# linhthi/BLISS-GNN

Hardware: AMD Instinct MI355X
Metric: steps/sec (train step: sample_blocks + gather + SAGE fwd/bwd + Adam + exp3), reddit-like (higher is better)
Workload: dtype bf16

## Files before the change

bliss_gnn_amd/csrc/sage.hip:

```cpp
#include "common.cuh"
#include "bliss_gnn.h"
#include <cstdlib>

namespace {

typedef __bf16 bf16x8_t __attribute__((ext_vector_type(8)));
typedef float f32x16_t __attribute__((ext_vector_type(16)));

#define TG_TPB 512
#define TG_M 32
#define TG_WAVES (TG_TPB / 64)
#define TG_NB (256 / 32 / TG_WAVES)

struct TileGemm {
  const bf16_t* a1; long long a1_stride; const int* ids;
  const bf16_t* w1; long long w1_stride; int k1;
  const bf16_t* a2; long long a2_stride; const bf16_t* w2; long long w2_stride; int k2;
  const bf16_t* bias;
  int m_bound; const int* m_dev; int n;
  bf16_t* out; long long out_stride;
  bf16_t* a_copy; long long copy_stride;
  bf16_t* in_norm; bf16_t* out_norm;
  int relu; unsigned drop_thresh; float drop_scale; unsigned seed; unsigned long long* ctr;
};

__device__ __forceinline__ int k_pad16(int k) { return (k + 15) & ~15; }
__device__ __host__ __forceinline__ int lds_stride(int k) {
  return ((k + 15) & ~15) + 8;
}

__device__ __forceinline__ uint32_t tg_drop_hash(uint32_t seed, uint32_t ctr, uint32_t idx) {
  uint32_t x = idx * 0x9e3779b1u + seed;
  x ^= ctr * 0x85ebca77u + 0x165667b1u;
  x ^= x >> 16; x *= 0x7feb352du; x ^= x >> 15; x *= 0x846ca68bu; x ^= x >> 16;
  x += ctr; x ^= x >> 15; x *= 0x2c1b3c6du; x ^= x >> 12;
  return x;
}

__device__ __forceinline__ float row_sumsq(const bf16_t* sh, int dim, int vec4, int lane) {
  float s = 0.f;
  if (vec4) {
    for (int c = lane * 4; c < dim; c += 256) {
      const float a = bf2f(sh[c]), b = bf2f(sh[c + 1]), cc = bf2f(sh[c + 2]), d = bf2f(sh[c + 3]);
      s += a * a; s += b * b; s += cc * cc; s += d * d;
    }
  } else {
    for (int c = lane; c < dim; c += 64) { const float a = bf2f(sh[c]); s += a * a; }
  }
  for (int d = 32; d >= 1; d >>= 1) s += __shfl_xor(s, d);
  return s;
}

__device__ __forceinline__ void rows_norm(const bf16_t* tile, int stride, int dim, int row0, int M, int m_bound, bf16_t* __restrict__ out,
                                          int wave, int lane) {
  constexpr int RPW = TG_M / TG_WAVES;
  float s[RPW];
#pragma unroll
  for (int q = 0; q < RPW; ++q) s[q] = 0.f;
  if (dim % 4 == 0) {
    for (int c = lane * 4; c < dim; c += 256)
#pragma unroll
      for (int q = 0; q < RPW; ++q) {
        const bf16_t* sh = tile + (size_t)(q * TG_WAVES + wave) * stride + c;
        const float a = bf2f(sh[0]), b = bf2f(sh[1]), cc = bf2f(sh[2]), d = bf2f(sh[3]);
        s[q] += a * a; s[q] += b * b; s[q] += cc * cc; s[q] += d * d;
      }
  } else {
    for (int c = lane; c < dim; c += 64)
#pragma unroll
      for (int q = 0; q < RPW; ++q) { const float a = bf2f(tile[(size_t)(q * TG_WAVES + wave) * stride + c]); s[q] += a * a; }
  }
  for (int d = 32; d >= 1; d >>= 1)
#pragma unroll
    for (int q = 0; q < RPW; ++q) s[q] += __shfl_xor(s[q], d);
#pragma unroll
  for (int q = 0; q < RPW; ++q) {
    const int r = row0 + q * TG_WAVES + wave;
    if (lane == 0 && r < m_bound) out[r] = r < M ? f2bf(sqrtf(s[q])) : (bf16_t)0;
  }
}

__device__ __forceinline__ void stage_rows(const bf16_t* __restrict__ a, long long a_stride, const int* row_id, int k,
                                           int row0, int m_bound, bf16_t* tile, int stride, bf16_t* __restrict__ copy, long long copy_stride,
                                           int wave, int lane) {
  const int kp = k_pad16(k);
  const bool even = (k % 2 == 0) && (a_stride % 2 == 0) && (((uintptr_t)a) % 4 == 0);
  const bool copy32 = copy && (copy_stride % 2 == 0) && (((uintptr_t)copy) % 4 == 0);
  if (even) {
    const int dw = k / 2;
    constexpr int MAXC = (1024 / 2 + 63) / 64;
    constexpr int RPW = TG_M / TG_WAVES, HALF = RPW;
#pragma unroll
    for (int hb = 0; hb < 1; ++hb) {
      uint32_t v[HALF][MAXC];
#pragma unroll
      for (int q = 0; q < HALF; ++q) {
        const int id = row_id[(hb * HALF + q) * TG_WAVES + wave];
        const uint32_t* src = reinterpret_cast<const uint32_t*>(a + (long long)(id < 0 ? 0 : id) * a_stride);
#pragma unroll
        for (int j = 0; j < MAXC; ++j) {
          const int c = lane + 64 * j;
          const uint32_t x = src[c < dw ? c : dw - 1];
          v[q][j] = (id >= 0 && c < dw) ? x : 0u;
        }
      }
#pragma unroll
      for (int q = 0; q < HALF; ++q) {
        const int lr = (hb * HALF + q) * TG_WAVES + wave, r = row0 + lr;
        uint32_t* sh = reinterpret_cast<uint32_t*>(tile + (size_t)lr * stride);
#pragma unroll
        for (int j = 0; j < MAXC; ++j) {
          const int c = lane + 64 * j;
          if (c < kp / 2) sh[c] = v[q][j];
          if (copy && r < m_bound && c < dw) {
            if (copy32) reinterpret_cast<uint32_t*>(copy + (long long)r * copy_stride)[c] = v[q][j];
            else { bf16_t* cp = copy + (long long)r * copy_stride + 2 * c; cp[0] = (bf16_t)(v[q][j] & 0xffffu); cp[1] = (bf16_t)(v[q][j] >> 16); }
          }
        }
      }
    }
  } else {
    for (int rd = 0; rd < TG_M / TG_WAVES; ++rd) {
      const int lr = rd * TG_WAVES + wave, r = row0 + lr, id = row_id[lr];
      const bf16_t* src = a + (long long)(id < 0 ? 0 : id) * a_stride;
      bf16_t* sh = tile + (size_t)lr * stride;
      for (int c = lane; c < kp; c += 64) {
        const bf16_t x = (id >= 0 && c < k) ? src[c] : (bf16_t)0;
        sh[c] = x;
        if (copy && r < m_bound && c < k) copy[(long long)r * copy_stride + c] = x;
      }
    }
  }
}

#define TG_SLAB 64
#define TG_WSTRIDE (TG_SLAB + 8)
#define TG_WROWS 256
typedef uint32_t u32x4_a4 __attribute__((ext_vector_type(4), aligned(4)));

struct WRegs { uint4 v[TG_WROWS * TG_SLAB / 8 / TG_TPB]; };

__device__ __forceinline__ void w_slab_load_full(WRegs& g, const bf16_t* __restrict__ w, long long w_stride, int N, int slab, int tid) {
  const int part = tid & 7, k = slab * TG_SLAB + 8 * part;
#pragma unroll
  for (int i = 0; i < (int)(sizeof(g.v) / sizeof(g.v[0])); ++i) {
    int n = i * (TG_TPB / 8) + (tid >> 3);
    n = n < N ? n : N - 1;
    const u32x4_a4 q = *reinterpret_cast<const u32x4_a4*>(w + (long long)n * w_stride + k);
    g.v[i] = make_uint4(q[0], q[1], q[2], q[3]);
  }
}
__device__ __forceinline__ void w_slab_load_tail(WRegs& g, const bf16_t* __restrict__ w, long long w_stride, int N, int K, int slab, int tid) {
  const int part = tid & 7, k = slab * TG_SLAB + 8 * part;
  for (int i = 0; i < (int)(sizeof(g.v) / sizeof(g.v[0])); ++i) {
    int n = i * (TG_TPB / 8) + (tid >> 3);
    n = n < N ? n : N - 1;
    const bf16_t* p = w + (long long)n * w_stride + k;
    union { uint4 u; bf16_t e[8]; } t;
    t.u = make_uint4(0, 0, 0, 0);
    for (int j = 0; j < 8; ++j) if (k + j < K) t.e[j] = p[j];
    g.v[i] = t.u;
  }
}
__device__ __forceinline__ int w_full_slabs(const bf16_t* w, long long w_stride, int K) {
  return ((w_stride % 2 == 0) && (((uintptr_t)w) % 4 == 0)) ? K / TG_SLAB : 0;
}
__device__ __forceinline__ void w_slab_store(const WRegs& g, bf16_t* wl, int tid) {
  const int part = tid & 7;
#pragma unroll
  for (int i = 0; i < (int)(sizeof(g.v) / sizeof(g.v[0])); ++i) {
    const int n = i * (TG_TPB / 8) + (tid >> 3);
    *reinterpret_cast<uint4*>(wl + (size_t)n * TG_WSTRIDE + 8 * part) = g.v[i];
  }
}

__device__ __forceinline__ void mma_product(WRegs& ga, WRegs& gb, const bf16_t* tile, int stride, int k, const bf16_t* __restrict__ w,
                                            long long w_stride, int n0, int N, bf16_t* wl, int tid, int lane, f32x16_t acc[TG_NB]) {
  const int kp = k_pad16(k), r = lane & 31, h = lane >> 5;
  const int nslab = (kp + TG_SLAB - 1) / TG_SLAB;
  auto multiply = [&](int sl) {
    if (n0 < N) {
#pragma unroll
      for (int st = 0; st < TG_SLAB / 16; ++st) {
        const int ks = sl * TG_SLAB + 16 * st;
        if (ks < kp) {
          const bf16x8_t a = *reinterpret_cast<const bf16x8_t*>(tile + (size_t)r * stride + ks + 8 * h);
#pragma unroll
          for (int nb = 0; nb < TG_NB; ++nb) {
            const bf16x8_t b = *reinterpret_cast<const bf16x8_t*>(wl + (size_t)(n0 + 32 * nb + r) * TG_WSTRIDE + 16 * st + 8 * h);
            acc[nb] = __builtin_amdgcn_mfma_f32_32x32x16_bf16(a, b, acc[nb], 0, 0, 0);
          }
        }
      }
    }
  };
  const int nfull = w_full_slabs(w, w_stride, k);
  for (int sl = 0; sl < nfull; sl += 2) {
    __syncthreads();
    w_slab_store(ga, wl, tid);
    if (sl + 2 < nfull) w_slab_load_full(ga, w, w_stride, N, sl + 2, tid);
    __syncthreads();
    multiply(sl);
    if (sl + 1 < nfull) {
      __syncthreads();
      w_slab_store(gb, wl, tid);
      if (sl + 3 < nfull) w_slab_load_full(gb, w, w_stride, N, sl + 3, tid);
      __syncthreads();
      multiply(sl + 1);
    }
  }
  for (int sl = nfull; sl < nslab; ++sl) {
    WRegs t;
    w_slab_load_tail(t, w, w_stride, N, k, sl, tid);
    __syncthreads();
    w_slab_store(t, wl, tid);
    __syncthreads();
    multiply(sl);
  }
}

__device__ __forceinline__ void tile_gemm_body(const TileGemm& p, bf16_t* lds, int* row_id, int dbg) {
  const int tid = threadIdx.x, wave = tid >> 6, lane = tid & 63;
  int M = p.m_bound;
  if (p.m_dev) { const int t = *p.m_dev; M = t < M ? t : M; }
  const int row0 = blockIdx.x * TG_M;
  const uint32_t ctr = p.drop_thresh ? (uint32_t)__hip_atomic_load(p.ctr, __ATOMIC_RELAXED, __HIP_MEMORY_SCOPE_AGENT) : 0u;
  const int N = p.n;
  if (row0 >= p.m_bound) return;
  if (row0 >= M) {
    for (int lr = wave; lr < TG_M; lr += TG_WAVES) {
      const int r = row0 + lr;
      if (r >= p.m_bound) break;
      for (int c = lane; c < N; c += 64) p.out[(long long)r * p.out_stride + c] = 0;
      if (p.a_copy) for (int c = lane; c < p.k1; c += 64) p.a_copy[(long long)r * p.copy_stride + c] = 0;
      if (lane == 0) { if (p.in_norm) p.in_norm[r] = 0; if (p.out_norm) p.out_norm[r] = 0; }
    }
    return;
  }
  const int s1 = lds_stride(p.k1), s2 = p.k2 ? lds_stride(p.k2) : 0;
  bf16_t* t1 = lds;
  bf16_t* t2 = lds + (size_t)TG_M * s1;
  const int n0 = wave * 32 * TG_NB;
  bf16_t* wl = lds + (size_t)TG_M * (s1 + s2);
  float bias_v[TG_NB];
#pragma unroll
  for (int nb = 0; nb < TG_NB; ++nb) bias_v[nb] = 0.f;
#pragma unroll
  for (int nb = 0; nb < TG_NB; ++nb) { const int col = n0 + 32 * nb + (lane & 31); if (p.bias && col < N) bias_v[nb] = bf2f(p.bias[col]); }
  WRegs ga, gb;
  {
    const int nf = w_full_slabs(p.w1, p.w1_stride, p.k1);
    if (nf > 0) w_slab_load_full(ga, p.w1, p.w1_stride, N, 0, tid);
    if (nf > 1) w_slab_load_full(gb, p.w1, p.w1_stride, N, 1, tid);
  }
  if (tid < TG_M) {
    const int r = row0 + tid;
    row_id[tid] = r < M ? (p.ids ? p.ids[r] : r) : -1;
    row_id[TG_M + tid] = r < M ? r : -1;
  }
  __syncthreads();
  if (!(dbg & 1)) stage_rows(p.a1, p.a1_stride, row_id, p.k1, row0, p.m_bound, t1, s1, p.a_copy, p.copy_stride, wave, lane);
  if (p.k2) stage_rows(p.a2, p.a2_stride, row_id + TG_M, p.k2, row0, p.m_bound, t2, s2, nullptr, 0, wave, lane);
  __syncthreads();
  if (p.in_norm && !(dbg & 4)) rows_norm(t1, s1, p.k1, row0, M, p.m_bound, p.in_norm, wave, lane);
  f32x16_t acc[TG_NB];
#pragma unroll
  for (int m = 0; m < TG_NB; ++m)
#pragma unroll
    for (int i = 0; i < 16; ++i) acc[m][i] = 0.f;
  if (!(dbg & 2)) mma_product(ga, gb, t1, s1, p.k1, p.w1, p.w1_stride, n0, N, wl, tid, lane, acc);
  if (p.k2) {
    const int nf = w_full_slabs(p.w2, p.w2_stride, p.k2);
    if (nf > 0) w_slab_load_full(ga, p.w2, p.w2_stride, N, 0, tid);
    if (nf > 1) w_slab_load_full(gb, p.w2, p.w2_stride, N, 1, tid);
    mma_product(ga, gb, t2, s2, p.k2, p.w2, p.w2_stride, n0, N, wl, tid, lane, acc);
  }
  __syncthreads();
  const int so = ((N + 63) & ~63) + 8;
  bf16_t* ot = lds;
  if (n0 < N) {
#pragma unroll
    for (int m = 0; m < TG_NB; ++m) {
      const int col = n0 + 32 * m + (lane & 31);
      const float bv = bias_v[m];
#pragma unroll
      for (int i = 0; i < 16; ++i) {
        const int lr = (i & 3) + 8 * (i >> 2) + 4 * (lane >> 5);
        float t = rbf(acc[m][i] + bv);
        if (p.relu) t = t > 0.f ? t : 0.f;
        if (p.drop_thresh) {
          const bool keep = tg_drop_hash(p.seed, ctr, (uint32_t)((row0 + lr) * N + col)) >= p.drop_thresh;
          t = keep ? rbf(t * p.drop_scale) : 0.f;
        }
        ot[(size_t)lr * so + col] = (row0 + lr < M && col < N) ? f2bf(t) : (bf16_t)0;
      }
    }
  }
  __syncthreads();
  const bool pair_ok = (N % 2 == 0) && (p.out_stride % 2 == 0) && (((uintptr_t)p.out) % 4 == 0);
  for (int lr = wave; lr < TG_M; lr += TG_WAVES) {
    const int r = row0 + lr;
    if (r >= p.m_bound) break;
    const bf16_t* sh = ot + (size_t)lr * so;
    bf16_t* o = p.out + (long long)r * p.out_stride;
    if (pair_ok) for (int c = lane * 2; c < N; c += 128) *reinterpret_cast<uint32_t*>(o + c) = *reinterpret_cast<const uint32_t*>(sh + c);
    else for (int c = lane; c < N; c += 64) o[c] = sh[c];
  }
  if (p.out_norm) rows_norm(ot, so, N, row0, M, p.m_bound, p.out_norm, wave, lane);
}

__global__ void __launch_bounds__(TG_TPB) k_tile_gemm(TileGemm p0, TileGemm p1, int n_sets, int dbg) {
  extern __shared__ __attribute__((aligned(16))) bf16_t tg_lds[];
  __shared__ int row_id[2 * TG_M];
  if (dbg & 8) return;
  tile_gemm_body(blockIdx.y == 0 ? p0 : p1, tg_lds, row_id, dbg);
  unsigned long long* ctr = p0.drop_thresh ? p0.ctr : (n_sets > 1 && p1.drop_thresh ? p1.ctr : nullptr);
  if (ctr) {
    __syncthreads();
    if (threadIdx.x == 0) {
      const unsigned long long total = (unsigned long long)gridDim.x * gridDim.y;
      if (atomicAdd(ctr + 1, 1ull) == total - 1) {
        __hip_atomic_store(ctr + 1, 0ull, __ATOMIC_RELAXED, __HIP_MEMORY_SCOPE_AGENT);
        atomicAdd(ctr, 1ull);
      }
    }
  }
}

bool convert(const bliss_tile_gemm_t* a, TileGemm* p, size_t* lds_bytes, int* tiles) {
  if (!a->a1 || !a->w1 || !a->out || a->k1 <= 0 || a->k1 > 1024 || a->n <= 0 || a->n > 256 || a->m_bound <= 0) return false;
  if (a->k2 < 0 || a->k2 > 1024 || (a->k2 > 0 && (!a->a2 || !a->w2))) return false;
  if (a->drop_p < 0.f || a->drop_p >= 1.f || (a->drop_p > 0.f && !a->drop_ctr)) return false;
  p->a1 = (const bf16_t*)a->a1; p->a1_stride = a->a1_stride; p->ids = a->ids;
  p->w1 = (const bf16_t*)a->w1; p->w1_stride = a->w1_stride; p->k1 = a->k1;
  p->a2 = (const bf16_t*)a->a2; p->a2_stride = a->a2_stride; p->w2 = (const bf16_t*)a->w2; p->w2_stride = a->w2_stride; p->k2 = a->k2;
  p->bias = (const bf16_t*)a->bias; p->m_bound = a->m_bound; p->m_dev = a->m_dev; p->n = a->n;
  p->out = (bf16_t*)a->out; p->out_stride = a->out_stride; p->a_copy = (bf16_t*)a->a_copy; p->copy_stride = a->copy_stride;
  p->in_norm = (bf16_t*)a->in_norm; p->out_norm = (bf16_t*)a->out_norm; p->relu = a->relu;
  p->drop_thresh = a->drop_p > 0.f ? (unsigned)((double)a->drop_p * 4294967296.0) : 0u;
  p->drop_scale = a->drop_p > 0.f ? 1.0f / (1.0f - a->drop_p) : 1.0f;
  p->seed = a->drop_seed; p->ctr = (unsigned long long*)a->drop_ctr;
  const size_t stage = ((size_t)TG_M * (lds_stride(a->k1) + (a->k2 ? lds_stride(a->k2) : 0)) + (size_t)TG_WROWS * TG_WSTRIDE) * sizeof(bf16_t);
  const size_t outt = (size_t)TG_M * (((a->n + 63) & ~63) + 8) * sizeof(bf16_t);
  *lds_bytes = stage > outt ? stage : outt;
  *tiles = (a->m_bound + TG_M - 1) / TG_M;
  return true;
}

}

extern "C" int bliss_tile_gemm(const bliss_tile_gemm_t* first, const bliss_tile_gemm_t* second, void* stream) {
  if (!first) return BLISS_EINVAL;
  TileGemm p0, p1;
  size_t l0 = 0, l1 = 0;
  int t0 = 0, t1 = 0;
  if (!convert(first, &p0, &l0, &t0)) return BLISS_EINVAL;
  p1 = p0;
  if (second && !convert(second, &p1, &l1, &t1)) return BLISS_EINVAL;
  const size_t lds = l0 > l1 ? l0 : l1;
  if (lds > 160 * 1024) return BLISS_EINVAL;
  static size_t lds_set = 0;
  if (lds > lds_set) {
    if (hipFuncSetAttribute((const void*)k_tile_gemm, hipFuncAttributeMaxDynamicSharedMemorySize, (int)lds) != hipSuccess) return BLISS_EINVAL;
    lds_set = lds;
  }
  const dim3 grid(t0 > t1 ? t0 : t1, second ? 2 : 1);
  static const int dbg = []() { const char* e = getenv("BLISS_TG_DEBUG"); return e ? atoi(e) : 0; }();
  k_tile_gemm<<<grid, TG_TPB, lds, (hipStream_t)stream>>>(p0, p1, second ? 2 : 1, dbg);
  return (int)hipGetLastError();
}
```

bliss_gnn_amd/csrc/sage_bwd.hip:

```cpp
#include "common.cuh"
#include "bliss_gnn.h"
#include <cstdlib>

namespace {

typedef __bf16 bf16x8_t __attribute__((ext_vector_type(8)));
typedef short s16x4_t __attribute__((ext_vector_type(4)));
typedef short s16x8_t __attribute__((ext_vector_type(8)));
typedef float f32x16_t __attribute__((ext_vector_type(16)));
typedef uint32_t u32x4_a4 __attribute__((ext_vector_type(4), aligned(4)));

__device__ __forceinline__ s16x4_t lds_tr4(const bf16_t* p) {
  return __builtin_amdgcn_ds_read_tr16_b64_v4i16((__attribute__((address_space(3))) s16x4_t*)(p));
}
__device__ __forceinline__ bf16x8_t tr_frag(const bf16_t* img, int stride, int k0, int c0, int lane) {
  const int g = lane >> 4, i = lane & 15, q = i >> 2, p = i & 3;
  const bf16_t* a = img + (size_t)(k0 + 8 * (g >> 1) + q) * stride + c0 + 16 * (g & 1) + 4 * p;
  const s16x4_t lo = lds_tr4(a), hi = lds_tr4(a + 4 * (size_t)stride);
  s16x8_t v;
  v[0] = lo[0]; v[1] = lo[1]; v[2] = lo[2]; v[3] = lo[3]; v[4] = hi[0]; v[5] = hi[1]; v[6] = hi[2]; v[7] = hi[3];
  return __builtin_bit_cast(bf16x8_t, v);
}

__device__ __forceinline__ uint4 ld16(const bf16_t* p) {
  const u32x4_a4 q = *reinterpret_cast<const u32x4_a4*>(p);
  return make_uint4(q[0], q[1], q[2], q[3]);
}
__device__ __forceinline__ uint4 ld8_masked(const bf16_t* p, int valid, bool aligned) {
  if (valid >= 8 && aligned) return ld16(p);
  union { uint4 u; bf16_t e[8]; } t;
  t.u = make_uint4(0, 0, 0, 0);
#pragma unroll
  for (int j = 0; j < 8; ++j) if (j < valid) t.e[j] = p[j];
  return t.u;
}

#define DG_TPB 512
#define DG_M 32
#define DG_SLAB 64
#define DG_WSTRIDE (256 + 32)

struct DGrad {
  const bf16_t* a1; long long a1_stride; const bf16_t* w1; long long w1_stride; int k1;
  const bf16_t* a2; long long a2_stride; const bf16_t* w2; long long w2_stride; int k2; int m2_bound; const int* m2_dev;
  int m_bound; const int* m_dev; int n;
  bf16_t* out; long long out_stride;
};

__device__ __host__ __forceinline__ int dg_astride(int k) { return ((k + 15) & ~15) + 8; }

__device__ __forceinline__ void dg_stage_a(const bf16_t* __restrict__ a, long long a_stride, int k, int row0, int M, bf16_t* tile, int tid) {
  const int kp = (k + 15) & ~15, st = dg_astride(k), chunks = kp / 8;
  const bool al = (a_stride % 2 == 0) && (((uintptr_t)a) % 4 == 0);
  for (int idx = tid; idx < DG_M * chunks; idx += DG_TPB) {
    const int lr = idx / chunks, c8 = idx - lr * chunks, r = row0 + lr;
    const uint4 v = r < M ? ld8_masked(a + (long long)r * a_stride + 8 * c8, k - 8 * c8, al) : make_uint4(0, 0, 0, 0);
    *reinterpret_cast<uint4*>(tile + (size_t)lr * st + 8 * c8) = v;
  }
}

__device__ __forceinline__ void dg_stage_w(const bf16_t* __restrict__ w, long long w_stride, int K, int N, int n0, int slab, bf16_t* wl, int tid) {
  const bool al = (w_stride % 2 == 0) && (((uintptr_t)w) % 4 == 0) && (n0 % 2 == 0);
  for (int idx = tid; idx < DG_SLAB * 32; idx += DG_TPB) {
    const int kr = idx >> 5, c8 = idx & 31, k = slab * DG_SLAB + kr, n = n0 + 8 * c8;
    const uint4 v = k < K ? ld8_masked(w + (long long)k * w_stride + n, N - n, al) : make_uint4(0, 0, 0, 0);
    *reinterpret_cast<uint4*>(wl + (size_t)kr * DG_WSTRIDE + 8 * c8) = v;
  }
}

__device__ __forceinline__ void dg_product(const bf16_t* tile, int k, const bf16_t* __restrict__ w, long long w_stride, int N, int n0,
                                           bf16_t* wl, int tid, int lane, int wave, f32x16_t& acc) {
  const int st = dg_astride(k), kp = (k + 15) & ~15, r = lane & 31, h = lane >> 5;
  const int nslab = (kp + DG_SLAB - 1) / DG_SLAB;
  for (int sl = 0; sl < nslab; ++sl) {
    __syncthreads();
    dg_stage_w(w, w_stride, k, N, n0, sl, wl, tid);
    __syncthreads();
#pragma unroll
    for (int s = 0; s < DG_SLAB / 16; ++s) {
      const int ks = sl * DG_SLAB + 16 * s;
      if (ks < kp) {
        const bf16x8_t a = *reinterpret_cast<const bf16x8_t*>(tile + (size_t)r * st + ks + 8 * h);
        const bf16x8_t b = tr_frag(wl, DG_WSTRIDE, 16 * s, 32 * wave, lane);
        acc = __builtin_amdgcn_mfma_f32_32x32x16_bf16(a, b, acc, 0, 0, 0);
      }
    }
  }
}

__global__ void __launch_bounds__(DG_TPB) k_dgrad(DGrad p) {
  extern __shared__ __attribute__((aligned(16))) bf16_t dg_lds[];
  const int tid = threadIdx.x, wave = tid >> 6, lane = tid & 63;
  int M = p.m_bound;
  if (p.m_dev) { const int t = *p.m_dev; M = t < M ? t : M; }
  int M2 = p.k2 ? p.m2_bound : 0;
  if (p.k2 && p.m2_dev) { const int t = *p.m2_dev; M2 = t < M2 ? t : M2; }
  if (M2 > M) M2 = M;
  const int row0 = blockIdx.x * DG_M, n0 = blockIdx.y * 256, N = p.n;
  if (row0 >= p.m_bound) return;
  const bool pair_ok = (p.out_stride % 2 == 0) && (((uintptr_t)p.out) % 4 == 0) && (N % 2 == 0);
  if (row0 >= M) {
    for (int idx = tid; idx < DG_M * 256; idx += DG_TPB) {
      const int r = row0 + (idx >> 8), c = n0 + (idx & 255);
      if (r < p.m_bound && c < N) p.out[(long long)r * p.out_stride + c] = 0;
    }
    return;
  }
  const int s1 = dg_astride(p.k1), s2 = p.k2 ? dg_astride(p.k2) : 0;
  bf16_t* t1 = dg_lds;
  bf16_t* t2 = t1 + (size_t)DG_M * s1;
  bf16_t* wl = t2 + (size_t)DG_M * s2;
  dg_stage_a(p.a1, p.a1_stride, p.k1, row0, M, t1, tid);
  const bool second = p.k2 && row0 < M2;
  if (second) dg_stage_a(p.a2, p.a2_stride, p.k2, row0, M2, t2, tid);
  f32x16_t acc;
#pragma unroll
  for (int i = 0; i < 16; ++i) acc[i] = 0.f;
  dg_product(t1, p.k1, p.w1, p.w1_stride, N, n0, wl, tid, lane, wave, acc);
  if (second) dg_product(t2, p.k2, p.w2, p.w2_stride, N, n0, wl, tid, lane, wave, acc);
  __syncthreads();
  const int so = 256 + 8;
  bf16_t* ot = dg_lds;
  {
    const int col = 32 * wave + (lane & 31);
#pragma unroll
    for (int i = 0; i < 16; ++i) {
      const int lr = (i & 3) + 8 * (i >> 2) + 4 * (lane >> 5);
      ot[(size_t)lr * so + col] = (row0 + lr < M) ? f2bf(acc[i]) : (bf16_t)0;
    }
  }
  __syncthreads();
  for (int lr = wave; lr < DG_M; lr += DG_TPB / 64) {
    const int r = row0 + lr;
    if (r >= p.m_bound) break;
    const bf16_t* sh = ot + (size_t)lr * so;
    bf16_t* o = p.out + (long long)r * p.out_stride + n0;
    const int nn = min(256, N - n0);
    if (pair_ok && (n0 % 2 == 0)) { for (int c = lane * 2; c < nn; c += 128) *reinterpret_cast<uint32_t*>(o + c) = *reinterpret_cast<const uint32_t*>(sh + c); }
    else for (int c = lane; c < nn; c += 64) o[c] = sh[c];
  }
}

#define WG_TPB 512
#define WG_ROWS 32
#define WG_TN 128
#define WG_DSTRIDE (256 + 32)
#define WG_XSTRIDE (WG_TN + 32)
#define WG_MAX_PROBS 2

struct WGradProb {
  const bf16_t* d; long long d_stride; int n_out;
  const bf16_t* x; long long x_stride; int k_in;
  int rows_bound; const int* rows_dev;
  bf16_t* dw; long long dw_stride; bf16_t* db;
  int col_tiles, chunks, rows_per_chunk; long long part_off;
  int ldp;
  int wg_begin;
};
struct WGradLaunch { WGradProb p[WG_MAX_PROBS]; int n; };

struct WRegsB { uint4 d[2]; uint4 x; };

__device__ __forceinline__ void wg_load(WRegsB& g, const WGradProb& p, int r_lo, int r_hi, int c0, int tid, bool d_al, bool x_al) {
#pragma unroll
  for (int i = 0; i < 2; ++i) {
    const int idx = tid + i * WG_TPB, lr = idx >> 5, c8 = idx & 31, r = r_lo + lr, n = 8 * c8;
    g.d[i] = (r < r_hi) ? ld8_masked(p.d + (long long)r * p.d_stride + n, p.n_out - n, d_al) : make_uint4(0, 0, 0, 0);
  }
  {
    const int lr = tid >> 4, c8 = tid & 15, r = r_lo + lr, c = c0 + 8 * c8;
    g.x = (r < r_hi) ? ld8_masked(p.x + (long long)r * p.x_stride + c, p.k_in - c, x_al) : make_uint4(0, 0, 0, 0);
  }
}
__device__ __forceinline__ void wg_store(const WRegsB& g, bf16_t* dimg, bf16_t* ximg, int tid) {
#pragma unroll
  for (int i = 0; i < 2; ++i) {
    const int idx = tid + i * WG_TPB, lr = idx >> 5, c8 = idx & 31;
    *reinterpret_cast<uint4*>(dimg + (size_t)lr * WG_DSTRIDE + 8 * c8) = g.d[i];
  }
  *reinterpret_cast<uint4*>(ximg + (size_t)(tid >> 4) * WG_XSTRIDE + 8 * (tid & 15)) = g.x;
}

__global__ void __launch_bounds__(WG_TPB) k_wgrad(WGradLaunch L, float* __restrict__ part) {
  __shared__ __attribute__((aligned(16))) bf16_t dimg[WG_ROWS * WG_DSTRIDE];
  __shared__ __attribute__((aligned(16))) bf16_t ximg[WG_ROWS * WG_XSTRIDE];
  const int tid = threadIdx.x, wave = tid >> 6, lane = tid & 63;
  const int pi = (L.n > 1 && (int)blockIdx.x >= L.p[1].wg_begin) ? 1 : 0;
  const WGradProb& p = L.p[pi];
  const int w = (int)blockIdx.x - p.wg_begin;
  const int ct = w % p.col_tiles, ch = w / p.col_tiles;
  int R = p.rows_bound;
  if (p.rows_dev) { const int t = *p.rows_dev; R = t < R ? t : R; }
  const int r_lo = ch * p.rows_per_chunk, r_hi = min(R, r_lo + p.rows_per_chunk);
  if (r_lo >= r_hi) return;
  const int c0 = ct * WG_TN;
  const int wm = wave >> 1, wn = wave & 1;
  const int m0 = 64 * wm, nl0 = 64 * wn;
  const bool m_act = m0 < p.n_out;
  const bool bias = p.db != nullptr && ct == 0 && wn == 0;
  f32x16_t acc[2][2], accb[2];
#pragma unroll
  for (int a = 0; a < 2; ++a) {
#pragma unroll
    for (int i = 0; i < 16; ++i) { acc[a][0][i] = 0.f; acc[a][1][i] = 0.f; accb[a][i] = 0.f; }
  }
  s16x8_t ones_s;
#pragma unroll
  for (int j = 0; j < 8; ++j) ones_s[j] = (short)0x3f80;
  const bf16x8_t ones = __builtin_bit_cast(bf16x8_t, ones_s);
  const bool d_al = (p.d_stride % 2 == 0) && (((uintptr_t)p.d) % 4 == 0);
  const bool x_al = (p.x_stride % 2 == 0) && (((uintptr_t)p.x) % 4 == 0);
  WRegsB g;
  wg_load(g, p, r_lo, r_hi, c0, tid, d_al, x_al);
  for (int rs = r_lo; rs < r_hi; rs += WG_ROWS) {
    __syncthreads();
    wg_store(g, dimg, ximg, tid);
    if (rs + WG_ROWS < r_hi) wg_load(g, p, rs + WG_ROWS, r_hi, c0, tid, d_al, x_al);
    __syncthreads();
    if (m_act) {
#pragma unroll
      for (int ks = 0; ks < WG_ROWS; ks += 16) {
        const bf16x8_t a0 = tr_frag(dimg, WG_DSTRIDE, ks, m0, lane), a1 = tr_frag(dimg, WG_DSTRIDE, ks, m0 + 32, lane);
        const bf16x8_t b0 = tr_frag(ximg, WG_XSTRIDE, ks, nl0, lane), b1 = tr_frag(ximg, WG_XSTRIDE, ks, nl0 + 32, lane);
        acc[0][0] = __builtin_amdgcn_mfma_f32_32x32x16_bf16(a0, b0, acc[0][0], 0, 0, 0);
        acc[0][1] = __builtin_amdgcn_mfma_f32_32x32x16_bf16(a0, b1, acc[0][1], 0, 0, 0);
        acc[1][0] = __builtin_amdgcn_mfma_f32_32x32x16_bf16(a1, b0, acc[1][0], 0, 0, 0);
        acc[1][1] = __builtin_amdgcn_mfma_f32_32x32x16_bf16(a1, b1, acc[1][1], 0, 0, 0);
        if (bias) {
          accb[0] = __builtin_amdgcn_mfma_f32_32x32x16_bf16(a0, ones, accb[0], 0, 0, 0);
          accb[1] = __builtin_amdgcn_mfma_f32_32x32x16_bf16(a1, ones, accb[1], 0, 0, 0);
        }
      }
    }
  }
  if (!m_act) return;
  float* pt = part + p.part_off + (long long)ch * 256 * p.ldp;
#pragma unroll
  for (int a = 0; a < 2; ++a) {
#pragma unroll
    for (int i = 0; i < 16; ++i) {
      const int n = m0 + 32 * a + (i & 3) + 8 * (i >> 2) + 4 * (lane >> 5);
      float* row = pt + (long long)n * p.ldp;
      row[c0 + nl0 + (lane & 31)] = acc[a][0][i];
      row[c0 + nl0 + 32 + (lane & 31)] = acc[a][1][i];
      if (bias && (lane & 31) == 0) row[p.col_tiles * WG_TN] = accb[a][i];
    }
  }
}

__global__ void __launch_bounds__(256) k_wgrad_reduce(WGradLaunch L, const float* __restrict__ part) {
  const int pi = blockIdx.y;
  const WGradProb& p = L.p[pi];
  int R = p.rows_bound;
  if (p.rows_dev) { const int t = *p.rows_dev; R = t < R ? t : R; }
  const int nch = R > 0 ? min(p.chunks, (R + p.rows_per_chunk - 1) / p.rows_per_chunk) : 0;
  const int q4 = (p.k_in + 3) / 4 + (p.db ? 1 : 0);
  const long long total = (long long)p.n_out * q4;
  const float* base = part + p.part_off;
  for (long long idx = (long long)blockIdx.x * 256 + threadIdx.x; idx < total; idx += (long long)gridDim.x * 256) {
    const int n = (int)(idx / q4), q = (int)(idx - (long long)n * q4);
    if (p.db && q == q4 - 1) {
      float s = 0.f;
      for (int c = 0; c < nch; ++c) s += base[((long long)c * 256 + n) * p.ldp + p.col_tiles * WG_TN];
      p.db[n] = f2bf(s);
      continue;
    }
    float4 s = make_float4(0.f, 0.f, 0.f, 0.f);
    for (int c = 0; c < nch; ++c) {
      const float4 v = *reinterpret_cast<const float4*>(base + ((long long)c * 256 + n) * p.ldp + 4 * q);
      s.x += v.x; s.y += v.y; s.z += v.z; s.w += v.w;
    }
    bf16_t* o = p.dw + (long long)n * p.dw_stride + 4 * q;
    const int left = p.k_in - 4 * q;
    o[0] = f2bf(s.x);
    if (left > 1) o[1] = f2bf(s.y);
    if (left > 2) o[2] = f2bf(s.z);
    if (left > 3) o[3] = f2bf(s.w);
  }
}

int wgrad_target_wgs() {
  static const int t = []() { const char* e = getenv("BLISS_WGRAD_WGS"); const int v = e ? atoi(e) : 0; return v > 0 ? v : 80; }();
  return t;
}

bool wgrad_plan(const bliss_wgrad_t* a, int n_probs, WGradLaunch* L, long long* floats, int* total_wgs) {
  if (n_probs < 1 || n_probs > WG_MAX_PROBS) return false;
  long long off = 0;
  int wgs = 0;
  int tiles_all = 0;
  for (int i = 0; i < n_probs; ++i) {
    if (!a[i].d || !a[i].x || !a[i].dw || a[i].n_out <= 0 || a[i].n_out > 256 || a[i].k_in <= 0 || a[i].rows_bound <= 0) return false;
    tiles_all += (a[i].k_in + WG_TN - 1) / WG_TN;
  }
  for (int i = 0; i < n_probs; ++i) {
    WGradProb& p = L->p[i];
    p.d = (const bf16_t*)a[i].d; p.d_stride = a[i].d_stride; p.n_out = a[i].n_out;
    p.x = (const bf16_t*)a[i].x; p.x_stride = a[i].x_stride; p.k_in = a[i].k_in;
    p.rows_bound = a[i].rows_bound; p.rows_dev = a[i].rows_dev;
    p.dw = (bf16_t*)a[i].dw; p.dw_stride = a[i].dw_stride; p.db = (bf16_t*)a[i].db;
    p.col_tiles = (a[i].k_in + WG_TN - 1) / WG_TN;
    int chunks = wgrad_target_wgs() / tiles_all;
    const int max_chunks = (a[i].rows_bound + 63) / 64;
    if (chunks > max_chunks) chunks = max_chunks;
    if (chunks < 1) chunks = 1;
    int rpc = (a[i].rows_bound + chunks - 1) / chunks;
    rpc = (rpc + WG_ROWS - 1) / WG_ROWS * WG_ROWS;
    chunks = (a[i].rows_bound + rpc - 1) / rpc;
    p.chunks = chunks; p.rows_per_chunk = rpc;
    p.ldp = p.col_tiles * WG_TN + 4;
    p.part_off = off;
    p.wg_begin = wgs;
    off += (long long)chunks * 256 * p.ldp;
    wgs += chunks * p.col_tiles;
  }
  L->n = n_probs;
  *floats = off;
  *total_wgs = wgs;
  return true;
}

int dgrad_launch(const bliss_dgrad_t* a, int k_max, void* stream) {
  if (!a || !a->a1 || !a->w1 || !a->out || a->k1 <= 0 || a->k1 > k_max || a->n <= 0 || a->m_bound <= 0) return BLISS_EINVAL;
  if (a->k2 < 0 || a->k2 > k_max || (a->k2 > 0 && (!a->a2 || !a->w2 || a->m2_bound <= 0))) return BLISS_EINVAL;
  DGrad p;
  p.a1 = (const bf16_t*)a->a1; p.a1_stride = a->a1_stride; p.w1 = (const bf16_t*)a->w1; p.w1_stride = a->w1_stride; p.k1 = a->k1;
  p.a2 = (const bf16_t*)a->a2; p.a2_stride = a->a2_stride; p.w2 = (const bf16_t*)a->w2; p.w2_stride = a->w2_stride; p.k2 = a->k2;
  p.m2_bound = a->m2_bound; p.m2_dev = a->m2_dev;
  p.m_bound = a->m_bound; p.m_dev = a->m_dev; p.n = a->n;
  p.out = (bf16_t*)a->out; p.out_stride = a->out_stride;
  const size_t stage = ((size_t)DG_M * (dg_astride(a->k1) + (a->k2 ? dg_astride(a->k2) : 0)) + (size_t)DG_SLAB * DG_WSTRIDE) * sizeof(bf16_t);
  const size_t outt = (size_t)DG_M * (256 + 8) * sizeof(bf16_t);
  const size_t lds = stage > outt ? stage : outt;
  if (lds > 160 * 1024) return BLISS_EINVAL;
  static size_t lds_set = 0;
  if (lds > lds_set) {
    if (hipFuncSetAttribute((const void*)k_dgrad, hipFuncAttributeMaxDynamicSharedMemorySize, (int)lds) != hipSuccess) return BLISS_EINVAL;
    lds_set = lds;
  }
  const dim3 grid((a->m_bound + DG_M - 1) / DG_M, (a->n + 255) / 256);
  k_dgrad<<<grid, DG_TPB, lds, (hipStream_t)stream>>>(p);
  return (int)hipGetLastError();
}

}

extern "C" {

int bliss_sage_dgrad(const bliss_dgrad_t* a, void* stream) { return dgrad_launch(a, 256, stream); }

int bliss_gat_dgrad(const bliss_dgrad_t* a, void* stream) { return dgrad_launch(a, 1024, stream); }

int64_t bliss_sage_wgrad_workspace(const bliss_wgrad_t* probs, int32_t n_probs) {
  WGradLaunch L;
  long long floats = 0;
  int wgs = 0;
  if (!probs || !wgrad_plan(probs, n_probs, &L, &floats, &wgs)) return -1;
  return (int64_t)floats;
}

int bliss_sage_wgrad(const bliss_wgrad_t* probs, int32_t n_probs, float* partials, int64_t partial_floats, void* stream) {
  WGradLaunch L;
  long long floats = 0;
  int wgs = 0;
  if (!probs || !partials || !wgrad_plan(probs, n_probs, &L, &floats, &wgs)) return BLISS_EINVAL;
  if (partial_floats < floats || (((uintptr_t)partials) % 16) != 0) return BLISS_EINVAL;
  hipStream_t st = (hipStream_t)stream;
  k_wgrad<<<wgs, WG_TPB, 0, st>>>(L, partials);
  int max_elems = 0;
  for (int i = 0; i < n_probs; ++i) { const int e = L.p[i].n_out * ((L.p[i].k_in + 3) / 4 + 1); if (e > max_elems) max_elems = e; }
  int gx = (max_elems + 255) / 256;
  if (gx > 1024) gx = 1024;
  k_wgrad_reduce<<<dim3(gx, n_probs), 256, 0, st>>>(L, partials);
  return (int)hipGetLastError();
}

}
```

Baseline: 1558.

## Vectorize and prefetch tail slabs and operands in SAGE forward and backward GEMMs

Forward tile GEMM now keeps the register double-buffered weight-slab pipeline running through the partial last slab when K is even, using clamped 32-bit loads and masked LDS stores instead of a scalar tail path. Backward dgrad gains 16-byte clamped loads with shift/zero fixup for the A tile and register-prefetched weight slabs. wgrad gets a deeper multi-buffer register prefetch of d/x rows. These target latency-bound global loads on odd-sized dims such as 41 and 602. The cost is extra register pressure and more complex boundary logic.

```diff
diff --git a/bliss_gnn_amd/csrc/sage.hip b/bliss_gnn_amd/csrc/sage.hip
--- a/bliss_gnn_amd/csrc/sage.hip
+++ b/bliss_gnn_amd/csrc/sage.hip
@@ -1,5 +1,6 @@
 #include "common.cuh"
 #include "bliss_gnn.h"
+#include "tile_tail.h"
 #include <cstdlib>
 
 namespace {
@@ -101,7 +102,7 @@
         for (int j = 0; j < MAXC; ++j) {
           const int c = lane + 64 * j;
           const uint32_t x = src[c < dw ? c : dw - 1];
-          v[q][j] = (id >= 0 && c < dw) ? x : 0u;
+          v[q][j] = x & ((id >= 0 && c < dw) ? 0xffffffffu : 0u);
         }
       }
 #pragma unroll
@@ -148,6 +149,22 @@
     n = n < N ? n : N - 1;
     const u32x4_a4 q = *reinterpret_cast<const u32x4_a4*>(w + (long long)n * w_stride + k);
     g.v[i] = make_uint4(q[0], q[1], q[2], q[3]);
+  }
+}
+__device__ __forceinline__ void w_slab_load_even(WRegs& g, const bf16_t* __restrict__ w, long long w_stride, int N, int K, int slab, int tid) {
+  const int part = tid & 7;
+  int e[4];
+#pragma unroll
+  for (int j = 0; j < 4; ++j) e[j] = tg_tail_elem(K, slab, part, j);
+#pragma unroll
+  for (int i = 0; i < (int)(sizeof(g.v) / sizeof(g.v[0])); ++i) {
+    int n = i * (TG_TPB / 8) + (tid >> 3);
+    n = n < N ? n : N - 1;
+    const bf16_t* row = w + (long long)n * w_stride;
+    uint32_t x[4];
+#pragma unroll
+    for (int j = 0; j < 4; ++j) x[j] = *reinterpret_cast<const uint32_t*>(row + e[j]);
+    g.v[i] = make_uint4(x[0], x[1], x[2], x[3]);
   }
 }
 __device__ __forceinline__ void w_slab_load_tail(WRegs& g, const bf16_t* __restrict__ w, long long w_stride, int N, int K, int slab, int tid) {
@@ -162,8 +179,13 @@
     g.v[i] = t.u;
   }
 }
-__device__ __forceinline__ int w_full_slabs(const bf16_t* w, long long w_stride, int K) {
-  return ((w_stride % 2 == 0) && (((uintptr_t)w) % 4 == 0)) ? K / TG_SLAB : 0;
+__device__ __forceinline__ int w_pipe_slabs(const bf16_t* w, long long w_stride, int K) {
+  const bool aligned = (w_stride % 2 == 0) && (((uintptr_t)w) % 4 == 0);
+  return !aligned ? 0 : (K % 2 == 0 ? (K + TG_SLAB - 1) / TG_SLAB : K / TG_SLAB);
+}
+__device__ __forceinline__ void w_slab_request(WRegs& g, const bf16_t* __restrict__ w, long long w_stride, int N, int K, int sl, int tid) {
+  if (sl < K / TG_SLAB) w_slab_load_full(g, w, w_stride, N, sl, tid);
+  else w_slab_load_even(g, w, w_stride, N, K, sl, tid);
 }
 __device__ __forceinline__ void w_slab_store(const WRegs& g, bf16_t* wl, int tid) {
   const int part = tid & 7;
@@ -171,6 +193,17 @@
   for (int i = 0; i < (int)(sizeof(g.v) / sizeof(g.v[0])); ++i) {
     const int n = i * (TG_TPB / 8) + (tid >> 3);
     *reinterpret_cast<uint4*>(wl + (size_t)n * TG_WSTRIDE + 8 * part) = g.v[i];
+  }
+}
+__device__ __forceinline__ void w_slab_store_masked(const WRegs& g, bf16_t* wl, int K, int slab, int tid) {
+  const int part = tid & 7;
+  uint32_t m[4];
+#pragma unroll
+  for (int j = 0; j < 4; ++j) m[j] = tg_tail_mask(K, slab, part, j);
+#pragma unroll
+  for (int i = 0; i < (int)(sizeof(g.v) / sizeof(g.v[0])); ++i) {
+    const int n = i * (TG_TPB / 8) + (tid >> 3);
+    *reinterpret_cast<uint4*>(wl + (size_t)n * TG_WSTRIDE + 8 * part) = make_uint4(g.v[i].x & m[0], g.v[i].y & m[1], g.v[i].z & m[2], g.v[i].w & m[3]);
   }
 }
 
@@ -194,22 +227,22 @@
       }
     }
   };
-  const int nfull = w_full_slabs(w, w_stride, k);
-  for (int sl = 0; sl < nfull; sl += 2) {
+  const int npipe = w_pipe_slabs(w, w_stride, k);
+  for (int sl = 0; sl < npipe; sl += 2) {
     __syncthreads();
-    w_slab_store(ga, wl, tid);
-    if (sl + 2 < nfull) w_slab_load_full(ga, w, w_stride, N, sl + 2, tid);
+    w_slab_store_masked(ga, wl, k, sl, tid);
+    if (sl + 2 < npipe) w_slab_request(ga, w, w_stride, N, k, sl + 2, tid);
     __syncthreads();
     multiply(sl);
-    if (sl + 1 < nfull) {
+    if (sl + 1 < npipe) {
       __syncthreads();
-      w_slab_store(gb, wl, tid);
-      if (sl + 3 < nfull) w_slab_load_full(gb, w, w_stride, N, sl + 3, tid);
+      w_slab_store_masked(gb, wl, k, sl + 1, tid);
+      if (sl + 3 < npipe) w_slab_request(gb, w, w_stride, N, k, sl + 3, tid);
       __syncthreads();
       multiply(sl + 1);
     }
   }
-  for (int sl = nfull; sl < nslab; ++sl) {
+  for (int sl = npipe; sl < nslab; ++sl) {
     WRegs t;
     w_slab_load_tail(t, w, w_stride, N, k, sl, tid);
     __syncthreads();
@@ -249,9 +282,9 @@
   for (int nb = 0; nb < TG_NB; ++nb) { const int col = n0 + 32 * nb + (lane & 31); if (p.bias && col < N) bias_v[nb] = bf2f(p.bias[col]); }
   WRegs ga, gb;
   {
-    const int nf = w_full_slabs(p.w1, p.w1_stride, p.k1);
-    if (nf > 0) w_slab_load_full(ga, p.w1, p.w1_stride, N, 0, tid);
-    if (nf > 1) w_slab_load_full(gb, p.w1, p.w1_stride, N, 1, tid);
+    const int nf = w_pipe_slabs(p.w1, p.w1_stride, p.k1);
+    if (nf > 0) w_slab_request(ga, p.w1, p.w1_stride, N, p.k1, 0, tid);
+    if (nf > 1) w_slab_request(gb, p.w1, p.w1_stride, N, p.k1, 1, tid);
   }
   if (tid < TG_M) {
     const int r = row0 + tid;
@@ -270,9 +303,9 @@
     for (int i = 0; i < 16; ++i) acc[m][i] = 0.f;
   if (!(dbg & 2)) mma_product(ga, gb, t1, s1, p.k1, p.w1, p.w1_stride, n0, N, wl, tid, lane, acc);
   if (p.k2) {
-    const int nf = w_full_slabs(p.w2, p.w2_stride, p.k2);
-    if (nf > 0) w_slab_load_full(ga, p.w2, p.w2_stride, N, 0, tid);
-    if (nf > 1) w_slab_load_full(gb, p.w2, p.w2_stride, N, 1, tid);
+    const int nf = w_pipe_slabs(p.w2, p.w2_stride, p.k2);
+    if (nf > 0) w_slab_request(ga, p.w2, p.w2_stride, N, p.k2, 0, tid);
+    if (nf > 1) w_slab_request(gb, p.w2, p.w2_stride, N, p.k2, 1, tid);
     mma_product(ga, gb, t2, s2, p.k2, p.w2, p.w2_stride, n0, N, wl, tid, lane, acc);
   }
   __syncthreads();
diff --git a/bliss_gnn_amd/csrc/sage_bwd.hip b/bliss_gnn_amd/csrc/sage_bwd.hip
--- a/bliss_gnn_amd/csrc/sage_bwd.hip
+++ b/bliss_gnn_amd/csrc/sage_bwd.hip
@@ -35,6 +35,21 @@
   return t.u;
 }
 
+__device__ __forceinline__ int ld8_col(int n, int width) { return n + 8 <= width ? n : width - 8; }
+__device__ __forceinline__ uint4 ld8_fix(uint4 q, int n, int width, bool live) {
+  const int sh = (!live || n >= width) ? 4 : (n + 8 <= width ? 0 : (n - (width - 8)) / 2);
+  if (sh == 0) return q;
+  uint4 o;
+  o.x = sh == 1 ? q.y : (sh == 2 ? q.z : (sh == 3 ? q.w : 0u));
+  o.y = sh == 1 ? q.z : (sh == 2 ? q.w : 0u);
+  o.z = sh == 1 ? q.w : 0u;
+  o.w = 0u;
+  return o;
+}
+__device__ __forceinline__ bool ld8_fast(const bf16_t* p, long long stride, int width) {
+  return (stride % 2 == 0) && (((uintptr_t)p) % 4 == 0) && (width % 2 == 0) && width >= 8;
+}
+
 #define DG_TPB 512
 #define DG_M 32
 #define DG_SLAB 64
@@ -68,13 +83,58 @@
   }
 }
 
+__device__ __forceinline__ void dg_stage_a_fast(const bf16_t* __restrict__ a, long long a_stride, int k, int row0, int M, bf16_t* tile, int tid) {
+  const int kp = (k + 15) & ~15, st = dg_astride(k), chunks = kp / 8, total = DG_M * chunks;
+  constexpr int U = 4;
+  for (int base = tid; base < total + tid; base += U * DG_TPB) {
+    uint4 q[U];
+#pragma unroll
+    for (int i = 0; i < U; ++i) {
+      int idx = base + i * DG_TPB;
+      idx = idx < total ? idx : total - 1;
+      const int lr = idx / chunks, c8 = idx - lr * chunks, r = row0 + lr;
+      q[i] = ld16(a + (long long)(r < M ? r : M - 1) * a_stride + ld8_col(8 * c8, k));
+    }
+#pragma unroll
+    for (int i = 0; i < U; ++i) {
+      const int idx = base + i * DG_TPB;
+      if (idx < total) {
+        const int lr = idx / chunks, c8 = idx - lr * chunks;
+        *reinterpret_cast<uint4*>(tile + (size_t)lr * st + 8 * c8) = ld8_fix(q[i], 8 * c8, k, row0 + lr < M);
+      }
+    }
+  }
+}
+
+struct DRegs { uint4 v[DG_SLAB * 32 / DG_TPB]; };
+
+__device__ __forceinline__ void dg_w_load(DRegs& g, const bf16_t* __restrict__ w, long long w_stride, int K, int N, int n0, int slab, int tid) {
+#pragma unroll
+  for (int i = 0; i < (int)(sizeof(g.v) / sizeof(g.v[0])); ++i) {
+    const int idx = tid + i * DG_TPB, kr = idx >> 5, c8 = idx & 31, k = slab * DG_SLAB + kr, n = n0 + 8 * c8;
+    g.v[i] = ld16(w + (long long)(k < K ? k : K - 1) * w_stride + ld8_col(n, N));
+  }
+}
+__device__ __forceinline__ void dg_w_store(const DRegs& g, int K, int N, int n0, int slab, bf16_t* wl, int tid) {
+#pragma unroll
+  for (int i = 0; i < (int)(sizeof(g.v) / sizeof(g.v[0])); ++i) {
+    const int idx = tid + i * DG_TPB, kr = idx >> 5, c8 = idx & 31, k = slab * DG_SLAB + kr, n = n0 + 8 * c8;
+    *reinterpret_cast<uint4*>(wl + (size_t)kr * DG_WSTRIDE + 8 * c8) = ld8_fix(g.v[i], n, N, k < K);
+  }
+}
+
 __device__ __forceinline__ void dg_product(const bf16_t* tile, int k, const bf16_t* __restrict__ w, long long w_stride, int N, int n0,
-                                           bf16_t* wl, int tid, int lane, int wave, f32x16_t& acc) {
+                                           bf16_t* wl, int tid, int lane, int wave, f32x16_t& acc, DRegs& g, bool fast) {
   const int st = dg_astride(k), kp = (k + 15) & ~15, r = lane & 31, h = lane >> 5;
   const int nslab = (kp + DG_SLAB - 1) / DG_SLAB;
   for (int sl = 0; sl < nslab; ++sl) {
     __syncthreads();
-    dg_stage_w(w, w_stride, k, N, n0, sl, wl, tid);
+    if (fast) {
+      dg_w_store(g, k, N, n0, sl, wl, tid);
+      if (sl + 1 < nslab) dg_w_load(g, w, w_stride, k, N, n0, sl + 1, tid);
+    } else {
+      dg_stage_w(w, w_stride, k, N, n0, sl, wl, tid);
+    }
     __syncthreads();
 #pragma unroll
     for (int s = 0; s < DG_SLAB / 16; ++s) {
@@ -110,14 +170,25 @@
   bf16_t* t1 = dg_lds;
   bf16_t* t2 = t1 + (size_t)DG_M * s1;
   bf16_t* wl = t2 + (size_t)DG_M * s2;
-  dg_stage_a(p.a1, p.a1_stride, p.k1, row0, M, t1, tid);
+  DRegs g;
+  const bool w1_fast = ld8_fast(p.w1, p.w1_stride, N);
+  if (w1_fast) dg_w_load(g, p.w1, p.w1_stride, p.k1, N, n0, 0, tid);
+  if (ld8_fast(p.a1, p.a1_stride, p.k1)) dg_stage_a_fast(p.a1, p.a1_stride, p.k1, row0, M, t1, tid);
+  else dg_stage_a(p.a1, p.a1_stride, p.k1, row0, M, t1, tid);
   const bool second = p.k2 && row0 < M2;
-  if (second) dg_stage_a(p.a2, p.a2_stride, p.k2, row0, M2, t2, tid);
+  if (second) {
+    if (ld8_fast(p.a2, p.a2_stride, p.k2)) dg_stage_a_fast(p.a2, p.a2_stride, p.k2, row0, M2, t2, tid);
+    else dg_stage_a(p.a2, p.a2_stride, p.k2, row0, M2, t2, tid);
+  }
   f32x16_t acc;
 #pragma unroll
   for (int i = 0; i < 16; ++i) acc[i] = 0.f;
-  dg_product(t1, p.k1, p.w1, p.w1_stride, N, n0, wl, tid, lane, wave, acc);
-  if (second) dg_product(t2, p.k2, p.w2, p.w2_stride, N, n0, wl, tid, lane, wave, acc);
+  dg_product(t1, p.k1, p.w1, p.w1_stride, N, n0, wl, tid, lane, wave, acc, g, w1_fast);
+  if (second) {
+    const bool w2_fast = ld8_fast(p.w2, p.w2_stride, N);
+    if (w2_fast) dg_w_load(g, p.w2, p.w2_stride, p.k2, N, n0, 0, tid);
+    dg_product(t2, p.k2, p.w2, p.w2_stride, N, n0, wl, tid, lane, wave, acc, g, w2_fast);
+  }
   __syncthreads();
   const int so = 256 + 8;
   bf16_t* ot = dg_lds;
@@ -180,6 +251,31 @@
   }
   *reinterpret_cast<uint4*>(ximg + (size_t)(tid >> 4) * WG_XSTRIDE + 8 * (tid & 15)) = g.x;
 }
+
+__device__ __forceinline__ void wg_load_fast(WRegsB& g, const WGradProb& p, int r_lo, int r_hi, int c0, int tid) {
+#pragma unroll
+  for (int i = 0; i < 2; ++i) {
+    const int idx = tid + i * WG_TPB, lr = idx >> 5, c8 = idx & 31, r = r_lo + lr;
+    g.d[i] = ld16(p.d + (long long)(r < r_hi ? r : r_hi - 1) * p.d_stride + ld8_col(8 * c8, p.n_out));
+  }
+  {
+    const int lr = tid >> 4, c8 = tid & 15, r = r_lo + lr;
+    g.x = ld16(p.x + (long long)(r < r_hi ? r : r_hi - 1) * p.x_stride + ld8_col(c0 + 8 * c8, p.k_in));
+  }
+}
+__device__ __forceinline__ void wg_store_fast(const WRegsB& g, const WGradProb& p, int r_lo, int r_hi, int c0, bf16_t* dimg, bf16_t* ximg, int tid) {
+#pragma unroll
+  for (int i = 0; i < 2; ++i) {
+    const int idx = tid + i * WG_TPB, lr = idx >> 5, c8 = idx & 31;
+    *reinterpret_cast<uint4*>(dimg + (size_t)lr * WG_DSTRIDE + 8 * c8) = ld8_fix(g.d[i], 8 * c8, p.n_out, r_lo + lr < r_hi);
+  }
+  const int lr = tid >> 4, c8 = tid & 15;
+  *reinterpret_cast<uint4*>(ximg + (size_t)lr * WG_XSTRIDE + 8 * c8) = ld8_fix(g.x, c0 + 8 * c8, p.k_in, r_lo + lr < r_hi);
+}
+
+#ifndef WG_DEPTH
+#define WG_DEPTH 2
+#endif
 
 __global__ void __launch_bounds__(WG_TPB) k_wgrad(WGradLaunch L, float* __restrict__ part) {
   __shared__ __attribute__((aligned(16))) bf16_t dimg[WG_ROWS * WG_DSTRIDE];
@@ -210,13 +306,7 @@
   const bf16x8_t ones = __builtin_bit_cast(bf16x8_t, ones_s);
   const bool d_al = (p.d_stride % 2 == 0) && (((uintptr_t)p.d) % 4 == 0);
   const bool x_al = (p.x_stride % 2 == 0) && (((uintptr_t)p.x) % 4 == 0);
-  WRegsB g;
-  wg_load(g, p, r_lo, r_hi, c0, tid, d_al, x_al);
-  for (int rs = r_lo; rs < r_hi; rs += WG_ROWS) {
-    __syncthreads();
-    wg_store(g, dimg, ximg, tid);
-    if (rs + WG_ROWS < r_hi) wg_load(g, p, rs + WG_ROWS, r_hi, c0, tid, d_al, x_al);
-    __syncthreads();
+  auto multiply = [&]() {
     if (m_act) {
 #pragma unroll
       for (int ks = 0; ks < WG_ROWS; ks += 16) {
@@ -231,6 +321,43 @@
           accb[1] = __builtin_amdgcn_mfma_f32_32x32x16_bf16(a1, ones, accb[1], 0, 0, 0);
         }
       }
+    }
+  };
+  if (ld8_fast(p.d, p.d_stride, p.n_out) && ld8_fast(p.x, p.x_stride, p.k_in)) {
+    constexpr int D = WG_DEPTH;
+    const int nsteps = (r_hi - r_lo + WG_ROWS - 1) / WG_ROWS;
+    WRegsB g[D];
+#pragma unroll
+    for (int j = 0; j < D; ++j) wg_load_fast(g[j], p, r_lo + (j < nsteps ? j : nsteps - 1) * WG_ROWS, r_hi, c0, tid);
+    int s = 0;
+    for (; s + 2 * D <= nsteps; s += D) {
+#pragma unroll
+      for (int j = 0; j < D; ++j) {
+        __syncthreads();
+        wg_store_fast(g[j], p, r_lo + (s + j) * WG_ROWS, r_hi, c0, dimg, ximg, tid);
+        wg_load_fast(g[j], p, r_lo + (s + j + D) * WG_ROWS, r_hi, c0, tid);
+        __syncthreads();
+        multiply();
+      }
+    }
+#pragma unroll
+    for (int j = 0; j < 2 * D - 1; ++j) {
+      if (s + j >= nsteps) break;
+      __syncthreads();
+      wg_store_fast(g[j % D], p, r_lo + (s + j) * WG_ROWS, r_hi, c0, dimg, ximg, tid);
+      if (s + j + D < nsteps) wg_load_fast(g[j % D], p, r_lo + (s + j + D) * WG_ROWS, r_hi, c0, tid);
+      __syncthreads();
+      multiply();
+    }
+  } else {
+    WRegsB g;
+    wg_load(g, p, r_lo, r_hi, c0, tid, d_al, x_al);
+    for (int rs = r_lo; rs < r_hi; rs += WG_ROWS) {
+      __syncthreads();
+      wg_store(g, dimg, ximg, tid);
+      if (rs + WG_ROWS < r_hi) wg_load(g, p, rs + WG_ROWS, r_hi, c0, tid, d_al, x_al);
+      __syncthreads();
+      multiply();
     }
   }
   if (!m_act) return;
diff --git a/bliss_gnn_amd/csrc/tile_tail.h b/bliss_gnn_amd/csrc/tile_tail.h
--- /dev/null
+++ b/bliss_gnn_amd/csrc/tile_tail.h
@@ -0,0 +1,22 @@
+#pragma once
+
+#if defined(__HIPCC__) || defined(__CUDACC__)
+#define TG_TAIL_HD __host__ __device__
+#else
+#define TG_TAIL_HD
+#endif
+
+#define TG_TAIL_SLAB 64
+
+TG_TAIL_HD inline int tg_tail_k0(int slab, int part) { return slab * TG_TAIL_SLAB + 8 * part; }
+TG_TAIL_HD inline int tg_tail_valid(int K, int slab, int part) {
+  const int left = K - tg_tail_k0(slab, part);
+  return left < 0 ? 0 : (left > 8 ? 8 : left);
+}
+TG_TAIL_HD inline int tg_tail_elem(int K, int slab, int part, int j) {
+  const int e = tg_tail_k0(slab, part) + 2 * j;
+  return e < K - 2 ? e : K - 2;
+}
+TG_TAIL_HD inline unsigned tg_tail_mask(int K, int slab, int part, int j) {
+  return 2 * j < tg_tail_valid(K, slab, part) ? 0xffffffffu : 0u;
+}
diff --git a/scratch/bwdbench.py b/scratch/bwdbench.py
--- /dev/null
+++ b/scratch/bwdbench.py
@@ -0,0 +1,31 @@
+import sys, os, torch
+sys.path.insert(0, os.path.dirname(os.path.dirname(os.path.abspath(__file__))))
+from bliss_gnn_amd.nn import sage_dgrad, sage_wgrad
+dev = torch.device("cuda")
+g = torch.Generator().manual_seed(0)
+def timeit(fn, n=20):
+    st = torch.cuda.Stream()
+    with torch.cuda.stream(st):
+        for _ in range(3): fn()
+    torch.cuda.synchronize()
+    gr = torch.cuda.CUDAGraph()
+    with torch.cuda.graph(gr):
+        for _ in range(n): fn()
+    gr.replay(); torch.cuda.synchronize()
+    ts = []
+    for _ in range(5):
+        a, b = torch.cuda.Event(enable_timing=True), torch.cuda.Event(enable_timing=True)
+        a.record(); gr.replay(); b.record(); torch.cuda.synchronize()
+        ts.append(a.elapsed_time(b) / n * 1e3)
+    return min(ts), max(ts)
+def rnd(*s): return torch.randn(*s, generator=g).bfloat16().to(dev)
+for name, M, K1, K2, M2, N in (("dgrad out layer 41->256", 1900, 41, 41, 256, 256), ("dgrad hidden 256->256", 4900, 256, 256, 1900, 256)):
+    a1, w1, a2, w2 = rnd(M, K1), rnd(K1, N), rnd(M2, K2), rnd(K2, N)
+    lo, hi = timeit(lambda: sage_dgrad(a1, w1, M, 0, a2=a2, w2=w2, m2_bound=M2))
+    print(f"{name:32s} {lo:7.1f} .. {hi:7.1f} us")
+for name, probs in (("wgrad input 11100+4900 x256x602", [(11100, 256, 602, False), (4900, 256, 602, True)]),
+                    ("wgrad hidden 2 x 1900 x256x256", [(1900, 256, 256, False), (1900, 256, 256, True)]),
+                    ("wgrad out 1900+256 x41x256", [(1900, 41, 256, False), (256, 41, 256, True)])):
+    args = [(rnd(R, n), rnd(R, k), R, 0, b) for R, n, k, b in probs]
+    lo, hi = timeit(lambda: sage_wgrad(args))
+    print(f"{name:32s} {lo:7.1f} .. {hi:7.1f} us   (product + reduce)")
diff --git a/scratch/isa_waits.py b/scratch/isa_waits.py
--- /dev/null
+++ b/scratch/isa_waits.py
@@ -0,0 +1,63 @@
+import os, re, subprocess, sys, tempfile
+
+ROOT = os.path.dirname(os.path.dirname(os.path.abspath(__file__)))
+HIPCC = os.environ.get("HIPCC", "/opt/rocm/bin/hipcc")
+FLAGS = ["-O3", "-std=c++17", "--offload-arch=gfx950", "-ffp-contract=off", "-I" + os.path.join(ROOT, "include"),
+         "--cuda-device-only", "-S"]
+
+
+def assembly(src):
+    with tempfile.TemporaryDirectory() as d:
+        out = os.path.join(d, "k.s")
+        subprocess.run([HIPCC] + FLAGS + ["-o", out, src], check=True)
+        return open(out).read()
+
+
+def kernels(asm):
+    names = re.findall(r"^\s*\.amdhsa_kernel\s+(\S+)", asm, re.M)
+    lines = asm.splitlines()
+    for name in names:
+        start = next(i for i, l in enumerate(lines) if l.startswith(name + ":"))
+        end = next(i for i in range(start, len(lines)) if lines[i].strip().startswith(".end_amdhsa_kernel"))
+        tail = next((i for i in range(end, len(lines)) if lines[i].startswith("; Occupancy")), end)
+        body = lines[start:tail + 1]
+        insts = [l.split(";")[0].strip() for l in lines[start:end]]
+        insts = [l for l in insts if l and not l.startswith(".") and not l.endswith(":")]
+        yield name, insts, body
+
+
+def figures(insts, body):
+    loads = [i for i, l in enumerate(insts) if l.startswith("global_load") or l.startswith("buffer_load")]
+    at_once = 0
+    for i in loads:
+        for l in insts[i + 1:i + 4]:
+            if l.startswith("global_load") or l.startswith("buffer_load"):
+                break
+            if l.startswith("s_waitcnt") and "vmcnt(0)" in l:
+                at_once += 1
+                break
+    text = "\n".join(body)
+    def meta(key):
+        m = re.search(r"\.amdhsa_" + key + r"\s+(\d+)", text)
+        return int(m.group(1)) if m else -1
+    m = re.search(r"; NumVgprs: (\d+)", text)
+    a = re.search(r"; NumAgprs: (\d+)", text)
+    s = re.search(r"; ScratchSize: (\d+)", text)
+    return dict(loads=len(loads), waited_at_once=at_once, vgprs=int(m.group(1)) if m else -1, agprs=int(a.group(1)) if a else 0,
+                scratch=int(s.group(1)) if s else meta("private_segment_fixed_size"))
+
+
+def main():
+    src, want = sys.argv[1], sys.argv[2:]
+    print(f"{'kernel':48s} {'loads':>6s} {'at once':>8s} {'VGPR':>5s} {'AGPR':>5s} {'scratch':>8s}")
+    for name, insts, body in kernels(assembly(src)):
+        short = subprocess.run(["c++filt", name], capture_output=True, text=True).stdout.strip()
+        short = short.replace("(anonymous namespace)::", "").split("(")[0] or name
+        if want and not any(w in short for w in want):
+            continue
+        f = figures(insts, body)
+        print(f"{short[:48]:48s} {f['loads']:6d} {f['waited_at_once']:8d} {f['vgprs']:5d} {f['agprs']:5d} {f['scratch']:8d}")
+
+
+if __name__ == "__main__":
+    main()
diff --git a/scratch/launch_medians.py b/scratch/launch_medians.py
--- /dev/null
+++ b/scratch/launch_medians.py
@@ -0,0 +1,25 @@
+import csv, glob, re, sys
+from collections import defaultdict
+import numpy as np
+f = glob.glob(sys.argv[1] + '/*/*_kernel_trace.csv')[0]
+want = sys.argv[2:] or ['k_tile_gemm', 'k_dgrad', 'k_wgrad', 'k_seg_scan']
+rows = list(csv.DictReader(open(f)))
+rows.sort(key=lambda r: int(r['Start_Timestamp']))
+def short(n):
+    n = re.sub(r'\(anonymous namespace\)::', '', n); n = re.sub(r'^void ', '', n)
+    return re.split(r'[(<]', n)[0]
+marks = [i for i, r in enumerate(rows) if 'k_exp3_update_multi' in r['Kernel_Name']]
+marks = marks[len(marks) // 5:]
+dur = defaultdict(list)
+spans = []
+for a, b in zip(marks[:-1], marks[1:]):
+    seen = defaultdict(int)
+    spans.append((int(rows[b]['Start_Timestamp']) - int(rows[a]['Start_Timestamp'])) / 1e3)
+    for r in rows[a:b]:
+        k = short(r['Kernel_Name'])
+        if k in want:
+            dur[(k, seen[k])].append((int(r['End_Timestamp']) - int(r['Start_Timestamp'])) / 1e3)
+            seen[k] += 1
+print(f"steps {len(spans)} step span us median {np.median(spans):.1f}")
+for (k, i), d in sorted(dur.items()):
+    print(f"{k:16s} #{i} n={len(d):4d} median {np.median(d):7.2f} p10 {np.percentile(d, 10):7.2f} p90 {np.percentile(d, 90):7.2f}")
```

After: 1571, median of 6. About the same (+0.8%).
